# uclanlp/visualbert

Measured on NVIDIA H100. Metric: image-text pairs/sec fwd+bwd VisualBERT-base, higher is better.
Workload: dtype bf16

## Files before the change

### visualbert_b200/csrc/vb_attention_wgmma.cu

```cuda
#include "vb_attention.cuh"

namespace vb {

constexpr int kWgTile = kBlk * kHd * 2;

template <int NKB>
struct AttnSmem {
    static constexpr int FWD_BYTES = 3 * NKB * kWgTile + NKB * kBlk * 4 + 16 + 1024;
    static constexpr int BWD_BYTES = (4 * NKB + NKB * NKB) * kWgTile + NKB * kBlk * 4 + 16 + 1024;
};

__device__ __forceinline__ uint64_t tile_desc(uint32_t saddr) { return wgmma_desc_sw128(saddr, kWgTile, 1024); }

__device__ __forceinline__ unsigned long long keep_word(const AttnParams& p, unsigned bh, int q, int kb, int nkb, int t) {
    if (p.drop_scale == 0.f) return ~0ull;
    return p.keep[(static_cast<unsigned long long>(bh) * (nkb * kBlk) + q) * nkb + kb] >> (2 * t);
}

template <int NKB>
__device__ __forceinline__ void qk_block(float (&s)[32], uint32_t sQ, uint32_t sK, int wg, int kb) {
#pragma unroll
    for (int k = 0; k < kHd / 16; ++k)
        wgmma_m64n64k16_ss<0, 0>(s, tile_desc(sQ + wg * kWgTile + k * 32), tile_desc(sK + kb * kWgTile + k * 32), k > 0 ? 1u : 0u);
}
__device__ __forceinline__ void pack_afrag(uint32_t (&a)[4], const float (&x)[32], int kk) {
    a[0] = pack_bf16x2(x[8 * kk], x[8 * kk + 1]);
    a[1] = pack_bf16x2(x[8 * kk + 2], x[8 * kk + 3]);
    a[2] = pack_bf16x2(x[8 * kk + 4], x[8 * kk + 5]);
    a[3] = pack_bf16x2(x[8 * kk + 6], x[8 * kk + 7]);
}
__device__ __forceinline__ void store_rows(bf16* base, long long ld, int r0, int nrows, const float (&x)[32], int t, float mul0, float mul1) {
#pragma unroll
    for (int j = 0; j < 8; ++j) {
        const int col = 8 * j + 2 * t;
        if (r0 < nrows) *reinterpret_cast<uint32_t*>(base + static_cast<long long>(r0) * ld + col) = pack_bf16x2(x[4 * j] * mul0, x[4 * j + 1] * mul0);
        if (r0 + 8 < nrows)
            *reinterpret_cast<uint32_t*>(base + static_cast<long long>(r0 + 8) * ld + col) = pack_bf16x2(x[4 * j + 2] * mul1, x[4 * j + 3] * mul1);
    }
}
__device__ __forceinline__ void store_tile(uint32_t tile, int r, const float (&x)[32], int t) {
#pragma unroll
    for (int j = 0; j < 8; ++j) {
        st_shared_u32(tile + swz(r, j) + 4 * t, pack_bf16x2(x[4 * j], x[4 * j + 1]));
        st_shared_u32(tile + swz(r + 8, j) + 4 * t, pack_bf16x2(x[4 * j + 2], x[4 * j + 3]));
    }
}

template <int NKB, bool VL = false>
__global__ void __launch_bounds__(NKB * 128, 1)
attn_fwd_wgmma_kernel(const __grid_constant__ CUtensorMap tmQKV, const AttnParams p) {
    extern __shared__ uint8_t smem_raw[];
    const uint32_t raw = smem_u32(smem_raw);
    const uint32_t base = (raw + 1023u) & ~1023u;
    uint8_t* smem = smem_raw + (base - raw);
    const uint32_t sQ = base, sK = base + NKB * kWgTile, sV = base + 2 * NKB * kWgTile;
    float* sbias = reinterpret_cast<float*>(smem + 3 * NKB * kWgTile);
    const uint32_t bar = base + 3 * NKB * kWgTile + NKB * kBlk * 4;
    const int tid = threadIdx.x, wg = tid >> 7, warp = (tid >> 5) & 3, lane = tid & 31, g = lane >> 2, t = lane & 3;
    const int item = blockIdx.x, b = item / p.A, h = item % p.A;
    const unsigned bh = static_cast<unsigned>(item);
    const SeqSpan sp = seq_span<VL>(p, b, h);
    const int S = sp.len;
    const int nkv = VL ? (S + kBlk - 1) / kBlk : NKB;
    const int row0 = VL ? static_cast<int>(sp.row0) : b * S;
    if (VL && S == 0) return;

    if (tid == 0) {
        tma_prefetch_desc(&tmQKV);
        mbar_init(bar, 1);
        fence_barrier_init();
    }
    __syncthreads();
    pdl_trigger();
    pdl_wait();
    if (tid == 0) {
        mbar_arrive_expect_tx(bar, 3 * nkv * kWgTile);
#pragma unroll
        for (int m = 0; m < 3; ++m)
#pragma unroll
            for (int kb = 0; kb < NKB; ++kb)
                if (!VL || kb < nkv) tma_load_2d(base + (m * NKB + kb) * kWgTile, &tmQKV, bar, m * p.H + h * kHd, row0 + kb * kBlk);
    }
    for (int i = tid; i < NKB * kBlk; i += NKB * 128) sbias[i] = key_bias2<VL>(p, b, i, S);
    const int q0 = wg * kBlk + warp * 16 + g;
    unsigned long long keep[NKB][2];
#pragma unroll
    for (int kb = 0; kb < NKB; ++kb) {
        keep[kb][0] = keep_word(p, bh, q0, kb, NKB, t);
        keep[kb][1] = keep_word(p, bh, q0 + 8, kb, NKB, t);
    }
    __syncthreads();
    if (VL && wg >= nkv) return;
    mbar_wait(bar, 0);

    float s[NKB][32];
    wgmma_fence();
#pragma unroll
    for (int kb = 0; kb < NKB; ++kb)
        if (!VL || kb < nkv) qk_block<NKB>(s[kb], sQ, sK, wg, kb);
    wgmma_commit();
    wgmma_wait<0>();

    const float sc2 = p.scale * kLog2e;
    float mx[2] = {-INFINITY, -INFINITY};
#pragma unroll
    for (int kb = 0; kb < NKB; ++kb)
#pragma unroll
        for (int j = 0; j < 8; ++j) {
            if (VL && kb >= nkv) break;
            const float b0 = sbias[kb * kBlk + 8 * j + 2 * t], b1 = sbias[kb * kBlk + 8 * j + 2 * t + 1];
            s[kb][4 * j] = fmaf(s[kb][4 * j], sc2, b0); s[kb][4 * j + 1] = fmaf(s[kb][4 * j + 1], sc2, b1);
            s[kb][4 * j + 2] = fmaf(s[kb][4 * j + 2], sc2, b0); s[kb][4 * j + 3] = fmaf(s[kb][4 * j + 3], sc2, b1);
            mx[0] = fmaxf(mx[0], fmaxf(s[kb][4 * j], s[kb][4 * j + 1]));
            mx[1] = fmaxf(mx[1], fmaxf(s[kb][4 * j + 2], s[kb][4 * j + 3]));
        }
    float l[2] = {0.f, 0.f};
#pragma unroll
    for (int r = 0; r < 2; ++r) {
        mx[r] = fmaxf(mx[r], __shfl_xor_sync(0xffffffffu, mx[r], 1));
        mx[r] = fmaxf(mx[r], __shfl_xor_sync(0xffffffffu, mx[r], 2));
    }
#pragma unroll
    for (int kb = 0; kb < NKB; ++kb)
#pragma unroll
        for (int j = 0; j < 8; ++j)
#pragma unroll
            for (int c = 0; c < 4; ++c) {
                if (VL && kb >= nkv) break;
                const int r = c >> 1;
                float e = fast_ex2(s[kb][4 * j + c] - mx[r]);
                l[r] += e;
                if (!((keep[kb][r] >> (8 * j + (c & 1))) & 1ull)) e = 0.f;
                s[kb][4 * j + c] = e;
            }
#pragma unroll
    for (int r = 0; r < 2; ++r) {
        l[r] += __shfl_xor_sync(0xffffffffu, l[r], 1);
        l[r] += __shfl_xor_sync(0xffffffffu, l[r], 2);
    }

    uint32_t pa[NKB][4][4];
#pragma unroll
    for (int kb = 0; kb < NKB; ++kb)
#pragma unroll
        for (int kk = 0; kk < 4; ++kk)
            if (!VL || kb < nkv) pack_afrag(pa[kb][kk], s[kb], kk);
    float o[32];
    wgmma_fence();
#pragma unroll
    for (int kb = 0; kb < NKB; ++kb)
#pragma unroll
        for (int kk = 0; kk < 4; ++kk)
            if (!VL || kb < nkv)
                wgmma_m64n64k16_rs<1>(o, pa[kb][kk], tile_desc(sV + kb * kWgTile + kk * 2048), (kb > 0 || kk > 0) ? 1u : 0u);
    wgmma_commit();
    wgmma_wait<0>();

    const float dscale = p.drop_scale != 0.f ? p.drop_scale : 1.f;
    store_rows(p.ctx + (VL ? sp.row0 : static_cast<long long>(b) * S) * p.H + h * kHd, p.H, q0, S, o, t, dscale / l[0], dscale / l[1]);
    if (t == 0 && p.lse != nullptr) {
        float* lse = p.lse + (VL ? sp.stat0 : static_cast<long long>(item) * S);
        if (q0 < S) lse[q0] = (mx[0] + log2f(l[0])) * 0.6931471805599453f;
        if (q0 + 8 < S) lse[q0 + 8] = (mx[1] + log2f(l[1])) * 0.6931471805599453f;
    }
}

template <int NKB, bool VL = false>
__global__ void __launch_bounds__(NKB * 128, 1)
attn_bwd_wgmma_kernel(const __grid_constant__ CUtensorMap tmQKV, const __grid_constant__ CUtensorMap tmDO, const AttnParams p) {
    extern __shared__ uint8_t smem_raw[];
    const uint32_t raw = smem_u32(smem_raw);
    const uint32_t base = (raw + 1023u) & ~1023u;
    uint8_t* smem = smem_raw + (base - raw);
    const uint32_t sQ = base, sK = base + NKB * kWgTile, sV = base + 2 * NKB * kWgTile, sDO = base + 3 * NKB * kWgTile;
    const uint32_t sPS = base + 4 * NKB * kWgTile;
    float* sbias = reinterpret_cast<float*>(smem + (4 * NKB + NKB * NKB) * kWgTile);
    const uint32_t bar = base + (4 * NKB + NKB * NKB) * kWgTile + NKB * kBlk * 4;
    const int tid = threadIdx.x, wg = tid >> 7, warp = (tid >> 5) & 3, lane = tid & 31, g = lane >> 2, t = lane & 3;
    const int item = blockIdx.x, b = item / p.A, h = item % p.A;
    const unsigned bh = static_cast<unsigned>(item);
    const long long ld = 3LL * p.H;
    const SeqSpan sp = seq_span<VL>(p, b, h);
    const int S = sp.len;
    const int nkv = VL ? (S + kBlk - 1) / kBlk : NKB;
    const int row0 = VL ? static_cast<int>(sp.row0) : b * S;
    const long long stat0 = VL ? sp.stat0 : static_cast<long long>(item) * S;
    if (VL && S == 0) return;
    const bool wg_live = !VL || wg < nkv;

    if (tid == 0) {
        tma_prefetch_desc(&tmQKV);
        tma_prefetch_desc(&tmDO);
        mbar_init(bar, 1);
        fence_barrier_init();
    }
    __syncthreads();
    pdl_trigger();
    pdl_wait();
    if (tid == 0) {
        mbar_arrive_expect_tx(bar, 4 * nkv * kWgTile);
#pragma unroll
        for (int kb = 0; kb < NKB; ++kb) {
            if (VL && kb >= nkv) break;
#pragma unroll
            for (int m = 0; m < 3; ++m) tma_load_2d(base + (m * NKB + kb) * kWgTile, &tmQKV, bar, m * p.H + h * kHd, row0 + kb * kBlk);
            tma_load_2d(sDO + kb * kWgTile, &tmDO, bar, h * kHd, row0 + kb * kBlk);
        }
    }
    for (int i = tid; i < NKB * kBlk; i += NKB * 128) sbias[i] = key_bias2<VL>(p, b, i, S);
    const int r0 = warp * 16 + g;
    const int q0 = wg * kBlk + r0;
    float lse2[2], dr[2];
#pragma unroll
    for (int r = 0; r < 2; ++r) {
        const int q = q0 + 8 * r;
        lse2[r] = q < S ? p.lse[stat0 + q] * kLog2e : INFINITY;
        dr[r] = q < S ? p.drow[stat0 + q] : 0.f;
    }
    unsigned long long keep[NKB][2];
#pragma unroll
    for (int kb = 0; kb < NKB; ++kb) {
        keep[kb][0] = keep_word(p, bh, q0, kb, NKB, t);
        keep[kb][1] = keep_word(p, bh, q0 + 8, kb, NKB, t);
    }
    __syncthreads();
    mbar_wait(bar, 0);
    const float sc2 = p.scale * kLog2e;
    const float ds = p.drop_scale != 0.f ? p.drop_scale : 1.f;
    auto probs = [&](float (&s)[32], int kb) {
#pragma unroll
        for (int j = 0; j < 8; ++j)
#pragma unroll
            for (int c = 0; c < 4; ++c)
                s[4 * j + c] = fast_ex2(fmaf(s[4 * j + c], sc2, sbias[kb * kBlk + 8 * j + 2 * t + (c & 1)]) - lse2[c >> 1]);
    };
    auto kept = [&](int kb, int j, int c) { return ((keep[kb][c >> 1] >> (8 * j + (c & 1))) & 1ull) != 0; };
    bf16* dqkv = p.dqkv + (VL ? sp.row0 : static_cast<long long>(b) * S) * ld + h * kHd;

#pragma unroll
    for (int kb = 0; kb < NKB; ++kb) {
        if (VL && (!wg_live || kb >= nkv)) break;
        float s[32];
        wgmma_fence();
        qk_block<NKB>(s, sQ, sK, wg, kb);
        wgmma_commit();
        wgmma_wait<0>();
        probs(s, kb);
#pragma unroll
        for (int j = 0; j < 8; ++j)
#pragma unroll
            for (int c = 0; c < 4; ++c) s[4 * j + c] = kept(kb, j, c) ? s[4 * j + c] * ds : 0.f;
        store_tile(sPS + (wg * NKB + kb) * kWgTile, r0, s, t);
    }
    fence_proxy_async_smem();
    __syncthreads();
    if (wg_live) {
        float acc[32];
        wgmma_fence();
#pragma unroll
        for (int qb = 0; qb < NKB; ++qb)
#pragma unroll
            for (int kk = 0; kk < 4; ++kk)
                if (!VL || qb < nkv)
                    wgmma_m64n64k16_ss<1, 1>(acc, tile_desc(sPS + (qb * NKB + wg) * kWgTile + kk * 2048),
                                             tile_desc(sDO + qb * kWgTile + kk * 2048), (qb > 0 || kk > 0) ? 1u : 0u);
        wgmma_commit();
        wgmma_wait<0>();
        store_rows(dqkv + 2 * p.H, ld, q0, S, acc, t, 1.f, 1.f);
    }
    __syncthreads();

    float dq[32];
#pragma unroll
    for (int kb = 0; kb < NKB; ++kb) {
        if (VL && (!wg_live || kb >= nkv)) break;
        float s[32], dp[32];
        wgmma_fence();
        qk_block<NKB>(s, sQ, sK, wg, kb);
#pragma unroll
        for (int k = 0; k < kHd / 16; ++k)
            wgmma_m64n64k16_ss<0, 0>(dp, tile_desc(sDO + wg * kWgTile + k * 32), tile_desc(sV + kb * kWgTile + k * 32), k > 0 ? 1u : 0u);
        wgmma_commit();
        wgmma_wait<0>();
        probs(s, kb);
#pragma unroll
        for (int j = 0; j < 8; ++j)
#pragma unroll
            for (int c = 0; c < 4; ++c) {
                const float dpd = kept(kb, j, c) ? dp[4 * j + c] * ds : 0.f;
                s[4 * j + c] *= dpd - dr[c >> 1];
            }
        store_tile(sPS + (wg * NKB + kb) * kWgTile, r0, s, t);
        uint32_t pa[4][4];
#pragma unroll
        for (int kk = 0; kk < 4; ++kk) pack_afrag(pa[kk], s, kk);
        wgmma_fence();
#pragma unroll
        for (int kk = 0; kk < 4; ++kk)
            wgmma_m64n64k16_rs<1>(dq, pa[kk], tile_desc(sK + kb * kWgTile + kk * 2048), (kb > 0 || kk > 0) ? 1u : 0u);
        wgmma_commit();
        wgmma_wait<0>();
    }
    if (wg_live) store_rows(dqkv, ld, q0, S, dq, t, p.scale, p.scale);
    fence_proxy_async_smem();
    __syncthreads();
    if (wg_live) {
        float acc[32];
        wgmma_fence();
#pragma unroll
        for (int qb = 0; qb < NKB; ++qb)
#pragma unroll
            for (int kk = 0; kk < 4; ++kk)
                if (!VL || qb < nkv)
                    wgmma_m64n64k16_ss<1, 1>(acc, tile_desc(sPS + (qb * NKB + wg) * kWgTile + kk * 2048),
                                             tile_desc(sQ + qb * kWgTile + kk * 2048), (qb > 0 || kk > 0) ? 1u : 0u);
        wgmma_commit();
        wgmma_wait<0>();
        store_rows(dqkv + p.H, ld, q0, S, acc, t, p.scale, p.scale);
    }
}

template <int NKB, bool VL = false>
static int launch_fwd_wgmma(const AttnParams& p, const CUtensorMap& tq, cudaStream_t st) {
    auto kern = attn_fwd_wgmma_kernel<NKB, VL>;
    static int configured[kMaxDevices] = {0};
    VB_CHECK_CUDA(ensure_dyn_smem(kern, AttnSmem<NKB>::FWD_BYTES, configured));
    ProfScope ps(st, PROF_ATTN_FWD, 4.0 * p.B * p.A * p.S * p.S * kHd, 1);
    VB_CHECK_CUDA(launch_pdl(kern, dim3(p.B * p.A), dim3(NKB * 128), AttnSmem<NKB>::FWD_BYTES, st, tq, p));
    return 0;
}
template <int NKB, bool VL = false>
static int launch_bwd_wgmma(const AttnParams& p, const CUtensorMap& tq, const CUtensorMap& td, cudaStream_t st) {
    auto kern = attn_bwd_wgmma_kernel<NKB, VL>;
    static int configured[kMaxDevices] = {0};
    VB_CHECK_CUDA(ensure_dyn_smem(kern, AttnSmem<NKB>::BWD_BYTES, configured));
    ProfScope ps(st, PROF_ATTN_DKV, 10.0 * p.B * p.A * p.S * p.S * kHd, 1);
    VB_CHECK_CUDA(launch_pdl(kern, dim3(p.B * p.A), dim3(NKB * 128), AttnSmem<NKB>::BWD_BYTES, st, tq, td, p));
    return 0;
}

int attn_fwd_wgmma(const AttnParams& p, const AttnDropOffset& off, cudaStream_t st) {
    const int nkb = (p.S + kBlk - 1) / kBlk;
    int rc = attn_keep_mask(p, off, nkb, st);
    if (rc) return rc;
    CUtensorMap tq;
    const bool vl = p.cu_seqlens != nullptr;
    const uint64_t rows = vl ? static_cast<uint64_t>(p.total) : static_cast<uint64_t>(p.B) * p.S;
    rc = make_tmap_bf16(&tq, p.qkv, 3ull * p.H, rows, 3ull * p.H, kBlk);
    if (rc) return rc;
    if (vl) {
        if (nkb == 1) rc = launch_fwd_wgmma<1, true>(p, tq, st);
        else if (nkb == 2) rc = launch_fwd_wgmma<2, true>(p, tq, st);
        else rc = launch_fwd_wgmma<3, true>(p, tq, st);
    } else if (nkb == 1) rc = launch_fwd_wgmma<1>(p, tq, st);
    else if (nkb == 2) rc = launch_fwd_wgmma<2>(p, tq, st);
    else rc = launch_fwd_wgmma<3>(p, tq, st);
    if (rc) return rc;
    VB_CHECK_CUDA(cudaGetLastError());
    return 0;
}

int attn_bwd_wgmma(const AttnParams& p, cudaStream_t st, bool delta_ready) {
    const int nkb = (p.S + kBlk - 1) / kBlk;
    int rc = 0;
    if (!delta_ready) {
        rc = attn_delta(p, st);
        if (rc) return rc;
    }
    CUtensorMap tq, td;
    const bool vl = p.cu_seqlens != nullptr;
    const uint64_t rows = vl ? static_cast<uint64_t>(p.total) : static_cast<uint64_t>(p.B) * p.S;
    rc = make_tmap_bf16(&tq, p.qkv, 3ull * p.H, rows, 3ull * p.H, kBlk);
    if (rc) return rc;
    rc = make_tmap_bf16(&td, p.dctx, static_cast<uint64_t>(p.H), rows, static_cast<uint64_t>(p.H), kBlk);
    if (rc) return rc;
    if (vl) {
        if (nkb == 1) rc = launch_bwd_wgmma<1, true>(p, tq, td, st);
        else if (nkb == 2) rc = launch_bwd_wgmma<2, true>(p, tq, td, st);
        else rc = launch_bwd_wgmma<3, true>(p, tq, td, st);
    } else if (nkb == 1) rc = launch_bwd_wgmma<1>(p, tq, td, st);
    else if (nkb == 2) rc = launch_bwd_wgmma<2>(p, tq, td, st);
    else rc = launch_bwd_wgmma<3>(p, tq, td, st);
    if (rc) return rc;
    VB_CHECK_CUDA(cudaGetLastError());
    return 0;
}

}
```

Baseline: 4364.

## Split attention forward into per-query-block CTAs with staged TMA barriers

The forward attention kernel now launches one 128-thread CTA per (batch, head, query block) instead of one CTA holding all query blocks as warpgroups. Each CTA loads only its own Q tile plus all K and V tiles, and K tiles get their own mbarriers so QK^T can start as each tile lands, with V waited on just before PV. This shrinks shared memory per CTA so several CTAs can share an SM, at the cost of K/V being loaded redundantly by every query-block CTA. The backward kernel splits its single load barrier into three (Q/K, dO, V) so early phases can start before V arrives.

```diff
diff --git a/visualbert_b200/csrc/vb_attention_wgmma.cu b/visualbert_b200/csrc/vb_attention_wgmma.cu
--- a/visualbert_b200/csrc/vb_attention_wgmma.cu
+++ b/visualbert_b200/csrc/vb_attention_wgmma.cu
@@ -6,8 +6,8 @@
 
 template <int NKB>
 struct AttnSmem {
-    static constexpr int FWD_BYTES = 3 * NKB * kWgTile + NKB * kBlk * 4 + 16 + 1024;
-    static constexpr int BWD_BYTES = (4 * NKB + NKB * NKB) * kWgTile + NKB * kBlk * 4 + 16 + 1024;
+    static constexpr int FWD_BYTES = (2 * NKB + 1) * kWgTile + NKB * kBlk * 4 + 8 * (NKB + 1) + 1024;
+    static constexpr int BWD_BYTES = (4 * NKB + NKB * NKB) * kWgTile + NKB * kBlk * 4 + 24 + 1024;
 };
 
 __device__ __forceinline__ uint64_t tile_desc(uint32_t saddr) { return wgmma_desc_sw128(saddr, kWgTile, 1024); }
@@ -47,42 +47,48 @@
 }
 
 template <int NKB, bool VL = false>
-__global__ void __launch_bounds__(NKB * 128, 1)
+__global__ void __launch_bounds__(128, 3)
 attn_fwd_wgmma_kernel(const __grid_constant__ CUtensorMap tmQKV, const AttnParams p) {
     extern __shared__ uint8_t smem_raw[];
     const uint32_t raw = smem_u32(smem_raw);
     const uint32_t base = (raw + 1023u) & ~1023u;
     uint8_t* smem = smem_raw + (base - raw);
-    const uint32_t sQ = base, sK = base + NKB * kWgTile, sV = base + 2 * NKB * kWgTile;
-    float* sbias = reinterpret_cast<float*>(smem + 3 * NKB * kWgTile);
-    const uint32_t bar = base + 3 * NKB * kWgTile + NKB * kBlk * 4;
-    const int tid = threadIdx.x, wg = tid >> 7, warp = (tid >> 5) & 3, lane = tid & 31, g = lane >> 2, t = lane & 3;
-    const int item = blockIdx.x, b = item / p.A, h = item % p.A;
+    const uint32_t sQ = base, sK = base + kWgTile, sV = base + (NKB + 1) * kWgTile;
+    float* sbias = reinterpret_cast<float*>(smem + (2 * NKB + 1) * kWgTile);
+    const uint32_t bar = base + (2 * NKB + 1) * kWgTile + NKB * kBlk * 4;
+    const int tid = threadIdx.x, warp = tid >> 5, lane = tid & 31, g = lane >> 2, t = lane & 3;
+    const int item = blockIdx.x / NKB, qb = blockIdx.x % NKB, b = item / p.A, h = item % p.A;
     const unsigned bh = static_cast<unsigned>(item);
     const SeqSpan sp = seq_span<VL>(p, b, h);
     const int S = sp.len;
     const int nkv = VL ? (S + kBlk - 1) / kBlk : NKB;
     const int row0 = VL ? static_cast<int>(sp.row0) : b * S;
-    if (VL && S == 0) return;
+    if (VL && qb >= nkv) return;
 
     if (tid == 0) {
         tma_prefetch_desc(&tmQKV);
-        mbar_init(bar, 1);
+        for (int i = 0; i <= NKB; ++i) mbar_init(bar + 8 * i, 1);
         fence_barrier_init();
     }
     __syncthreads();
     pdl_trigger();
     pdl_wait();
     if (tid == 0) {
-        mbar_arrive_expect_tx(bar, 3 * nkv * kWgTile);
-#pragma unroll
-        for (int m = 0; m < 3; ++m)
-#pragma unroll
-            for (int kb = 0; kb < NKB; ++kb)
-                if (!VL || kb < nkv) tma_load_2d(base + (m * NKB + kb) * kWgTile, &tmQKV, bar, m * p.H + h * kHd, row0 + kb * kBlk);
-    }
-    for (int i = tid; i < NKB * kBlk; i += NKB * 128) sbias[i] = key_bias2<VL>(p, b, i, S);
-    const int q0 = wg * kBlk + warp * 16 + g;
+        mbar_arrive_expect_tx(bar, 2 * kWgTile);
+        tma_load_2d(sQ, &tmQKV, bar, h * kHd, row0 + qb * kBlk);
+#pragma unroll
+        for (int kb = 0; kb < NKB; ++kb) {
+            if (VL && kb >= nkv) break;
+            if (kb > 0) mbar_arrive_expect_tx(bar + 8 * kb, kWgTile);
+            tma_load_2d(sK + kb * kWgTile, &tmQKV, bar + 8 * kb, p.H + h * kHd, row0 + kb * kBlk);
+        }
+        mbar_arrive_expect_tx(bar + 8 * NKB, nkv * kWgTile);
+#pragma unroll
+        for (int kb = 0; kb < NKB; ++kb)
+            if (!VL || kb < nkv) tma_load_2d(sV + kb * kWgTile, &tmQKV, bar + 8 * NKB, 2 * p.H + h * kHd, row0 + kb * kBlk);
+    }
+    for (int i = tid; i < NKB * kBlk; i += 128) sbias[i] = key_bias2<VL>(p, b, i, S);
+    const int q0 = qb * kBlk + warp * 16 + g;
     unsigned long long keep[NKB][2];
 #pragma unroll
     for (int kb = 0; kb < NKB; ++kb) {
@@ -90,14 +96,15 @@
         keep[kb][1] = keep_word(p, bh, q0 + 8, kb, NKB, t);
     }
     __syncthreads();
-    if (VL && wg >= nkv) return;
-    mbar_wait(bar, 0);
 
     float s[NKB][32];
     wgmma_fence();
 #pragma unroll
     for (int kb = 0; kb < NKB; ++kb)
-        if (!VL || kb < nkv) qk_block<NKB>(s[kb], sQ, sK, wg, kb);
+        if (!VL || kb < nkv) {
+            mbar_wait(bar + 8 * kb, 0);
+            qk_block<NKB>(s[kb], sQ, sK, 0, kb);
+        }
     wgmma_commit();
     wgmma_wait<0>();
 
@@ -146,6 +153,7 @@
         for (int kk = 0; kk < 4; ++kk)
             if (!VL || kb < nkv) pack_afrag(pa[kb][kk], s[kb], kk);
     float o[32];
+    mbar_wait(bar + 8 * NKB, 0);
     wgmma_fence();
 #pragma unroll
     for (int kb = 0; kb < NKB; ++kb)
@@ -191,21 +199,27 @@
     if (tid == 0) {
         tma_prefetch_desc(&tmQKV);
         tma_prefetch_desc(&tmDO);
-        mbar_init(bar, 1);
+        for (int i = 0; i < 3; ++i) mbar_init(bar + 8 * i, 1);
         fence_barrier_init();
     }
     __syncthreads();
     pdl_trigger();
     pdl_wait();
     if (tid == 0) {
-        mbar_arrive_expect_tx(bar, 4 * nkv * kWgTile);
-#pragma unroll
-        for (int kb = 0; kb < NKB; ++kb) {
-            if (VL && kb >= nkv) break;
-#pragma unroll
-            for (int m = 0; m < 3; ++m) tma_load_2d(base + (m * NKB + kb) * kWgTile, &tmQKV, bar, m * p.H + h * kHd, row0 + kb * kBlk);
-            tma_load_2d(sDO + kb * kWgTile, &tmDO, bar, h * kHd, row0 + kb * kBlk);
-        }
+        mbar_arrive_expect_tx(bar, 2 * nkv * kWgTile);
+        mbar_arrive_expect_tx(bar + 8, nkv * kWgTile);
+        mbar_arrive_expect_tx(bar + 16, nkv * kWgTile);
+#pragma unroll
+        for (int m = 0; m < 2; ++m)
+#pragma unroll
+            for (int kb = 0; kb < NKB; ++kb)
+                if (!VL || kb < nkv) tma_load_2d(base + (m * NKB + kb) * kWgTile, &tmQKV, bar, m * p.H + h * kHd, row0 + kb * kBlk);
+#pragma unroll
+        for (int kb = 0; kb < NKB; ++kb)
+            if (!VL || kb < nkv) tma_load_2d(sDO + kb * kWgTile, &tmDO, bar + 8, h * kHd, row0 + kb * kBlk);
+#pragma unroll
+        for (int kb = 0; kb < NKB; ++kb)
+            if (!VL || kb < nkv) tma_load_2d(sV + kb * kWgTile, &tmQKV, bar + 16, 2 * p.H + h * kHd, row0 + kb * kBlk);
     }
     for (int i = tid; i < NKB * kBlk; i += NKB * 128) sbias[i] = key_bias2<VL>(p, b, i, S);
     const int r0 = warp * 16 + g;
@@ -256,6 +270,7 @@
     __syncthreads();
     if (wg_live) {
         float acc[32];
+        mbar_wait(bar + 8, 0);
         wgmma_fence();
 #pragma unroll
         for (int qb = 0; qb < NKB; ++qb)
@@ -270,6 +285,8 @@
     }
     __syncthreads();
 
+    mbar_wait(bar + 8, 0);
+    mbar_wait(bar + 16, 0);
     float dq[32];
 #pragma unroll
     for (int kb = 0; kb < NKB; ++kb) {
@@ -326,7 +343,7 @@
     static int configured[kMaxDevices] = {0};
     VB_CHECK_CUDA(ensure_dyn_smem(kern, AttnSmem<NKB>::FWD_BYTES, configured));
     ProfScope ps(st, PROF_ATTN_FWD, 4.0 * p.B * p.A * p.S * p.S * kHd, 1);
-    VB_CHECK_CUDA(launch_pdl(kern, dim3(p.B * p.A), dim3(NKB * 128), AttnSmem<NKB>::FWD_BYTES, st, tq, p));
+    VB_CHECK_CUDA(launch_pdl(kern, dim3(p.B * p.A * NKB), dim3(128), AttnSmem<NKB>::FWD_BYTES, st, tq, p));
     return 0;
 }
 template <int NKB, bool VL = false>
```

Result: no change. 4371 (median of 6 runs) (+0.2%).
